# BaZzz01010101/ReflaxMan

Measured on AMD Instinct MI355X. Metric: Mrays/sec at 3840×2160 depth-8; max per-channel |Δ| vs CPU reference, higher is better.
Workload: dtype f32; 1 GPU; C3 synth16: 16 spheres + 4 textured triangles + sun, 3840x2160, depth 8, 1 spp; scene=synth16, width=3840, height=2160, depth=8, spp=1, parallelism=single-gpu

## Files before the change

### include/rfx.h

```cpp
#ifndef RFX_H
#define RFX_H
#include <stddef.h>
#include <stdint.h>

#ifdef __cplusplus
extern "C" {
#endif

#define RFX_ABI_VERSION 5

typedef enum {
  RFX_OK = 0,
  RFX_ERR_ARG = -1,
  RFX_ERR_HIP = -2,
  RFX_ERR_STATE = -3,
  RFX_ERR_IO = -4,
  RFX_ERR_RNG = -5,
  RFX_ERR_NODEV = -6
} rfx_status;

enum { RFX_METAL = 0, RFX_DIELECTRIC = 1 };

typedef struct rfx_scene rfx_scene;
typedef struct rfx_renderer rfx_renderer;
// ... 17 lines not shown
int rfx_scene_plane_count(const rfx_scene *scene);
int rfx_triangle_set_texture(rfx_scene *scene, int object_index, int texture_index, const float uv[6]);
int rfx_scene_add_light(rfx_scene *scene, const float origin[3], float radius, const float rgb[3], float power);
int rfx_scene_add_texture_argb(rfx_scene *scene, uint32_t width, uint32_t height, const uint32_t *argb);
int rfx_scene_add_texture_file(rfx_scene *scene, const char *path, int *loaded);
int rfx_scene_set_skybox_file(rfx_scene *scene, const char *path);
int rfx_scene_set_skybox_argb(rfx_scene *scene, uint32_t width, uint32_t height, const uint32_t *argb);
int rfx_scene_counts(const rfx_scene *scene, int *spheres, int *triangles, int *lights, int *textures);
int rfx_scene_tri_bvh_dump(const rfx_scene *scene, int32_t counts[5], float *boxes, int32_t *children,
                           int32_t *leaf_ids, int32_t *residual);
int rfx_scene_cull_dump(const rfx_scene *scene, float recs[64 * 8], float tris[32 * 12], uint64_t *valid);
int rfx_scene_set_tri_mates(rfx_scene *scene, int on);
int rfx_scene_tri_mates(const rfx_scene *scene, int32_t *leader, float *plane);
int rfx_scene_set_far_lights(rfx_scene *scene, int mode);
int rfx_scene_far_light(const rfx_scene *scene, int light, float terms[8]);

void rfx_camera_view(const float eye[3], const float at[3], float view[9]);
float rfx_camera_rz(uint32_t width, float fov);

int rfx_tga_load(const char *path, uint32_t *width, uint32_t *height, uint32_t *argb, size_t capacity);
int rfx_tga_save(const char *path, uint32_t width, uint32_t height, const uint32_t *argb);
int rfx_bmp_save(const char *path, uint32_t width, uint32_t height, const uint32_t *argb);
void rfx_argb_from_rgb(const float *rgb, size_t pixels, uint32_t *argb);

int rfx_renderer_create(rfx_renderer **out, int device);
void rfx_renderer_destroy(rfx_renderer *r);
int rfx_renderer_device(const rfx_renderer *r);
int rfx_renderer_set_stream(rfx_renderer *r, void *hip_stream);
int rfx_renderer_set_scene(rfx_renderer *r, const rfx_scene *scene);
int rfx_renderer_set_tile_order(rfx_renderer *r, int mode);
// ... 190 lines not shown
```

### reflaxman_amd/_lib.py

```python
from __future__ import annotations

import ctypes as C
import os

from . import _build

RFX_OK = 0
RFX_NCOUNTERS = 40
RFX_ABI_VERSION = 5
RFX_ORDER_CELL_BITS, RFX_ORDER_DIR_BITS, RFX_ORDER_TILE = 4, 10, 4096
RFX_TRI_RECORD_WORDS = 41
METAL, DIELECTRIC = 0, 1

_fp = C.POINTER(C.c_float)
_u32p = C.POINTER(C.c_uint32)
_u64p = C.POINTER(C.c_uint64)


class RfxError(RuntimeError):
    pass


class Frame(C.Structure):
    _fields_ = [
# ... 39 lines not shown

SIGNATURES = [
    ("rfx_abi_version", C.c_int, []),
    ("rfx_last_error", C.c_char_p, []),
    ("rfx_build_options", C.c_int, []),
    ("rfx_scene_create", C.c_void_p, [C.c_float] * 4),
    ("rfx_scene_destroy", None, [C.c_void_p]),
    ("rfx_scene_add_sphere", C.c_int, [C.c_void_p, _fp, C.c_float, C.c_int, _fp, C.c_float, C.c_float]),
    ("rfx_scene_add_triangle", C.c_int, [C.c_void_p, _fp, _fp, _fp, C.c_int, _fp, C.c_float, C.c_float]),
    ("rfx_scene_add_mesh", C.c_int, [C.c_void_p, _fp, C.c_uint32, _u32p, C.c_uint32, C.c_int, _fp, C.c_float, C.c_float]),
    ("rfx_scene_tri_bvh_dump", C.c_int, [C.c_void_p, _i32p, _fp, _i32p, _i32p, _i32p]),
    ("rfx_scene_cull_dump", C.c_int, [C.c_void_p, _fp, _fp, _u64p]),
    ("rfx_scene_set_tri_mates", C.c_int, [C.c_void_p, C.c_int]),
    ("rfx_scene_tri_mates", C.c_int, [C.c_void_p, _i32p, _fp]),
    ("rfx_scene_set_far_lights", C.c_int, [C.c_void_p, C.c_int]),
    ("rfx_scene_far_light", C.c_int, [C.c_void_p, C.c_int, _fp]),
    ("rfx_scene_add_plane", C.c_int, [C.c_void_p, _fp, _fp, C.c_int, _fp, C.c_float, C.c_float]),
    ("rfx_scene_plane_count", C.c_int, [C.c_void_p]),
    ("rfx_triangle_set_texture", C.c_int, [C.c_void_p, C.c_int, C.c_int, _fp]),
    ("rfx_scene_add_light", C.c_int, [C.c_void_p, _fp, C.c_float, _fp, C.c_float]),
    ("rfx_scene_add_texture_argb", C.c_int, [C.c_void_p, C.c_uint32, C.c_uint32, _u32p]),
    ("rfx_scene_add_texture_file", C.c_int, [C.c_void_p, C.c_char_p, C.POINTER(C.c_int)]),
    ("rfx_scene_set_skybox_file", C.c_int, [C.c_void_p, C.c_char_p]),
    ("rfx_scene_set_skybox_argb", C.c_int, [C.c_void_p, C.c_uint32, C.c_uint32, _u32p]),
    ("rfx_scene_counts", C.c_int, [C.c_void_p] + [C.POINTER(C.c_int)] * 4),
    ("rfx_camera_view", None, [_fp, _fp, _fp]),
    ("rfx_camera_rz", C.c_float, [C.c_uint32, C.c_float]),
    ("rfx_tga_load", C.c_int, [C.c_char_p, _u32p, _u32p, _u32p, C.c_size_t]),
    ("rfx_tga_save", C.c_int, [C.c_char_p, C.c_uint32, C.c_uint32, _u32p]),
    ("rfx_bmp_save", C.c_int, [C.c_char_p, C.c_uint32, C.c_uint32, _u32p]),
# ... 197 lines not shown
```

### reflaxman_amd/csrc/rfx_bounce.h

```cpp
#pragma once
#include <hip/hip_runtime.h>

#include <cstddef>
#include <type_traits>

#include "rfx_math.h"
#include "rfx_types.h"
#include "rfx_shade_inputs.h"
#include "rfx_queries.h"

#pragma clang fp contract(off)

namespace rfx {

struct Park {
  int after;
  QRay *queue;
  uint32_t *count;
  uint32_t trace, out;
  static constexpr bool kRefill = false;
  __device__ __forceinline__ void ids(uint32_t &t, uint32_t &o) const { t = trace; o = out; }
  __device__ __forceinline__ uint32_t *keys() const { return nullptr; }
  __device__ __forceinline__ BvhGlobal bvh() const { return BvhGlobal{}; }
};
// ... 48 lines not shown
}

__device__ __forceinline__ bool near_light(const LightRec &L, v3 d)
{
  return fabsf(d.x) < L.near && fabsf(d.y) < L.near && fabsf(d.z) < L.near;
}

__device__ __forceinline__ LightRec reread_light(const LightRec *l, uint64_t when)
{
  typedef const __attribute__((address_space(4))) LightRec *ConstLightPtr;
  ConstLightPtr p = (ConstLightPtr)l;
  asm("" : "+s"(p) : "s"(when));
  return *(const LightRec *)p;
}

template <bool STATS, bool CULL, bool MANYL, bool SMALL, bool PLANES, bool PARK, class PK, bool ONEL = false,
          bool TBVH = false, bool FARL = false>
__device__ __forceinline__ col trace_from(const DevScene &RFX_SCENE_PARAM, v3 origin, v3 ray, col mulc, col pix, int refl,
                                          int depth, v3 rd, const float *lut, Cnt &cnt, bool valid, const PK &park,
                                          bool &parked, const uint64_t *pm_tile = nullptr, bool pm_shadow = true)
{
#ifdef RFX_LAUNDER_SCENE
  const DevScene &S = S_in;
#endif
  static_assert(!FARL || (ONEL && SMALL && CULL && !MANYL && !STATS), "FARL: the small-scene one-light culling kernels");
  constexpr bool FAR_SHADE = FARL && (RFX_FAR_LIGHT == 1 || RFX_FAR_LIGHT == 2);
  constexpr bool FAR_CONE = FARL && (RFX_FAR_LIGHT == 1 || RFX_FAR_LIGHT == 3);
  bool seg0 = pm_tile != nullptr;
  parked = false;
  if (valid && refl == 0) RFX_CNT(C_RAYS);
  const Tabs<SMALL> T{S};
  bool alive = valid && refl < depth;
  int occ_hint = -1;
#ifdef RFX_DEBUG_SEGS
  int nseg = 0;
#endif
  RFX_PROF_BEGIN(P_SEG);
  while (__ballot(alive))
  {
#ifdef RFX_DEBUG_SEGS
    if (alive) ++nseg;
#endif
// ... 56 lines not shown
    MatRec m{0.0f, 0.0f, 0.0f, 0.0f};
    int diel = 0;
    v3 reflv = mk(0.0f, 0.0f, 0.0f);
    float rayLen = 0.0f, normLen = 0.0f, reflectLen = 0.0f;
    col sumL = mkc(0.0f, 0.0f, 0.0f), sumS = mkc(0.0f, 0.0f, 0.0f);
    for (int base = 0;; base += 32)
    {
      RFX_PROF_BEGIN(P_SHADOW);
      uint32_t lit = 0;
      const int nl = ONEL ? 1 : min(32, S.n_light - base);
      for (int q = 0; q < nl; ++q)
      {
        const LightRec L = S.lights[base + q];
        bool facing = false;
        v3 sray = mk(0.0f, 0.0f, 0.0f);
        if (hit)
        {
          RFX_CNT(C_L_EVAL);
          const v3 dtl = sub(mk(L.ox, L.oy, L.oz), drop);
          if (dot(dtl, norm) > kVerySmall)
          {
            RFX_CNT(C_L_FACING);
            facing = true;
            sray = add(dtl, mul(rd, L.radius));
          }
        }
        if (__ballot(facing))
        {
          if constexpr (SMALL)
          {
            uint64_t om = S.cull_valid;
            if constexpr (CULL)
            {
              if (!MANYL && seg0 && pm_shadow && q < kPrimLights)
                om = pm_tile[1 + q];
              else
              {
                Bundle SB;
                bool far_cone = false;
                if constexpr (FAR_CONE) far_cone = __ballot(facing && !near_light(L, drop)) == 0;
                if (far_cone) SB = make_bundle_far(drop, L, facing);
                else SB = make_bundle(drop, sray, facing);
                if (SB.ok) om = cull_small(T.cull(), S.cull_valid, SB);
                RFX_CULL_STAT(1, SB.ok, __ballot(facing), om, S.cull_valid);
              }
            }
            if (facing && !occluded_small<STATS, PLANES>(S, drop, sray, skip_sph, skip_tri, skip_pln, om, cnt))
              lit |= 1u << q;
          }
          else
// ... 173 lines not shown
          alive = false;
        }
      }
    }
    if constexpr (PK::kRefill) park.refill(alive, origin, ray, mulc, pix, refl, rd);
  }
  RFX_PROF_END(P_SEG);
#ifdef RFX_DEBUG_SEGS
  return mkc((float)nseg, 0.0f, 0.0f);
#else
  return pix;
#endif
}

template <bool STATS, bool CULL, bool MANYL, bool SMALL, bool PLANES, bool ONEL = false, bool TBVH = false,
          bool FARL = false>
__device__ __forceinline__ col trace(const DevScene &S, v3 origin, v3 ray, int depth, v3 rd, const float *lut,
                                     Cnt &cnt, bool valid, const uint64_t *pm_tile = nullptr, bool pm_shadow = true)
{
  bool parked;
  return trace_from<STATS, CULL, MANYL, SMALL, PLANES, false, Park, ONEL, TBVH, FARL>(S, origin, ray, mkc(1.0f, 1.0f, 1.0f), mkc(0.0f, 0.0f, 0.0f), 0,
                                                       depth, rd, lut, cnt, valid, Park{0, nullptr, nullptr, 0, 0},
                                                       parked, pm_tile, pm_shadow);
}

}
```

### reflaxman_amd/csrc/rfx_bundle.h

```cpp
#pragma once
#include <hip/hip_runtime.h>

#include "rfx_math.h"
#include "rfx_types.h"

#pragma clang fp contract(off)

namespace rfx {

constexpr float kCullRel = 2e-3f;

struct Bundle {
  float cx, cy, cz, rw;
  float ax, ay, az, cosa, sina;
  bool ok;
};

__device__ __forceinline__ float lane_bcast(float v, int lane)
{
  return __int_as_float(__builtin_amdgcn_readlane(__float_as_int(v), lane));
}

__device__ __forceinline__ float wave_max_nonneg(float v)
{
  uint32_t u = __float_as_uint(v);
  u = max(u, (uint32_t)__builtin_amdgcn_update_dpp(0, (int)u, 0x111, 0xf, 0xf, false));
  u = max(u, (uint32_t)__builtin_amdgcn_update_dpp(0, (int)u, 0x112, 0xf, 0xf, false));
  u = max(u, (uint32_t)__builtin_amdgcn_update_dpp(0, (int)u, 0x114, 0xf, 0xf, false));
  u = max(u, (uint32_t)__builtin_amdgcn_update_dpp(0, (int)u, 0x118, 0xf, 0xf, false));
  u = max(u, (uint32_t)__builtin_amdgcn_update_dpp(0, (int)u, 0x142, 0xa, 0xf, false));
  u = max(u, (uint32_t)__builtin_amdgcn_update_dpp(0, (int)u, 0x143, 0xc, 0xf, false));
  return __int_as_float(__builtin_amdgcn_readlane((int)u, 63));
}

__device__ __forceinline__ float cdot(float ax, float ay, float az, float bx, float by, float bz)
{
#if RFX_CULL_FMA
  return __builtin_fmaf(az, bz, __builtin_fmaf(ay, by, ax * bx));
#else
  return ax * bx + ay * by + az * bz;
#endif
}

__device__ __forceinline__ Bundle make_bundle(v3 o, v3 d, bool live)
{
  Bundle B;
  const int ref = __ffsll((long long)__ballot(live)) - 1;
  B.cx = lane_bcast(o.x, ref); B.cy = lane_bcast(o.y, ref); B.cz = lane_bcast(o.z, ref);
  const float dx = lane_bcast(d.x, ref), dy = lane_bcast(d.y, ref), dz = lane_bcast(d.z, ref);
  const float inv = __builtin_amdgcn_rsqf(cdot(dx, dy, dz, dx, dy, dz));
  B.ax = dx * inv; B.ay = dy * inv; B.az = dz * inv;
  const float ex = o.x - B.cx, ey = o.y - B.cy, ez = o.z - B.cz;
  const float e2 = cdot(ex, ey, ez, ex, ey, ez);
  const float cosl = cdot(d.x, d.y, d.z, B.ax, B.ay, B.az) * __builtin_amdgcn_rsqf(cdot(d.x, d.y, d.z, d.x, d.y, d.z));
  const float dev = 1.0f - cosl;
  const bool bad = live && !(e2 <= 1.0e30f && dev >= -0.5f && dev <= 2.5f);
// ... 116 lines not shown
  const float px = B.cx + tp * B.ax - q.v0x, py = B.cy + tp * B.ay - q.v0y, pz = B.cz + tp * B.az - q.v0z;
  const float chord = __builtin_amdgcn_sqrtf(fmaxf(2.0f - 2.0f * B.cosa, 0.0f)) * 1.001f;
  const float R = (h * chord * (1.0f + ian) * ind + B.rw * (1.0f + ind) + 1e-4f * tp) * 1.001f + 1e-6f;
  const float cvx = B.cx - q.v0x, cvy = B.cy - q.v0y, cvz = B.cz - q.v0z;
  const float mag = __builtin_amdgcn_sqrtf(cvx * cvx + cvy * cvy + cvz * cvz) * 1.001f + B.rw + (h + B.rw) * ind;
  const float m = 1e-2f * mag + 1e-6f;
  const float u0 = q.gux * px + q.guy * py + q.guz * pz, v0 = q.gvx * px + q.gvy * py + q.gvz * pz;
  return u0 + (R + m) * q.nu < 0.0f || v0 + (R + m) * q.nv < 0.0f ||
         u0 + v0 - R * q.nuv - m * (q.nu + q.nv) > 1.0f;
}

template <bool FOOT = false>
__device__ __forceinline__ uint64_t cull_small(const CullRec *tab, uint64_t valid, const Bundle &B,
                                               const CullTri *ttab = nullptr)
{
  const CullRec g = tab[threadIdx.x & 63u];
  const float vx = g.x - B.cx, vy = g.y - B.cy, vz = g.z - B.cz;
  const float L2 = cdot(vx, vy, vz, vx, vy, vz);
  const float L = __builtin_amdgcn_sqrtf(L2);
#if RFX_CULL_FMA
  const float rp = __builtin_fmaf(kCullRel, L + B.rw, g.r + B.rw);
  const float va = cdot(vx, vy, vz, B.ax, B.ay, B.az);
  const float lim = __builtin_fmaf(B.cosa, __builtin_amdgcn_sqrtf(fmaxf(__builtin_fmaf(-rp, rp, L2), 0.0f)), -(B.sina * rp));
#else
  const float rp = g.r + B.rw + kCullRel * (L + B.rw);
  const float va = cdot(vx, vy, vz, B.ax, B.ay, B.az);
  const float lim = B.cosa * __builtin_amdgcn_sqrtf(fmaxf(L2 - rp * rp, 0.0f)) - B.sina * rp;
#endif
  const float side = cdot(g.nx, g.ny, g.nz, B.cx, B.cy, B.cz) - g.d;
  const float an = cdot(g.nx, g.ny, g.nz, B.ax, B.ay, B.az);
  const float ms = B.rw + 1e-3f * (L + g.r + B.rw) + 1e-6f, ma = B.sina + 1e-3f;
  const bool away = (side > ms && an > ma) || (side < -ms && an < -ma);
  bool keep = !(L > rp && va < lim) && !away;
  if constexpr (FOOT)
    if ((threadIdx.x & 63u) >= 32u && keep) keep = !tri_footprint_misses(ttab[(threadIdx.x & 63u) - 32u], side, an, B);
  return __ballot(keep) & valid;
}

__device__ __forceinline__ uint64_t all_bits(int n) { return n >= 64 ? ~0ull : ((1ull << n) - 1ull); }

__device__ __forceinline__ uint32_t pair_bits(uint64_t m)
{
  uint64_t x = (m | (m >> 1)) & 0x5555555555555555ull;
  x = (x | (x >> 1)) & 0x3333333333333333ull;
  x = (x | (x >> 2)) & 0x0F0F0F0F0F0F0F0Full;
  x = (x | (x >> 4)) & 0x00FF00FF00FF00FFull;
  x = (x | (x >> 8)) & 0x0000FFFF0000FFFFull;
  x = (x | (x >> 16)) & 0x00000000FFFFFFFFull;
  return (uint32_t)x;
}
// ... 3 lines not shown
```

### reflaxman_amd/csrc/rfx_config.h

```cpp
#pragma once

#ifndef RFX_DIV_FAST
#define RFX_DIV_FAST 1
#endif
#ifndef RFX_DIV_SINGLE
#define RFX_DIV_SINGLE 0
#endif

#ifndef RFX_BVH_LEAF_PAIRS
#define RFX_BVH_LEAF_PAIRS 4
#endif
#ifndef RFX_TRI_BVH
#define RFX_TRI_BVH 1
#endif
#ifndef RFX_TRI_BVH_LEAF
#define RFX_TRI_BVH_LEAF 4
#endif
#ifndef RFX_TRI_BVH_AUTO_MIN
#define RFX_TRI_BVH_AUTO_MIN 128
#endif
#ifndef RFX_TRI_BVH_NARROW_MIN
#define RFX_TRI_BVH_NARROW_MIN (1 << 30)
#endif

#if !defined(RFX_WAVES_PER_EU) && defined(RFX_LANES_WAVES_PER_EU) && defined(RFX_UNIT_LANES_FAST)
#define RFX_WAVES_PER_EU RFX_LANES_WAVES_PER_EU
#endif
#ifndef RFX_WAVES_PER_EU
#define RFX_WAVES_PER_EU 7
#endif
#ifndef RFX_WG_WAVES
#define RFX_WG_WAVES 2
#endif
#ifndef RFX_TRI_MATES
#define RFX_TRI_MATES 2
#endif
#ifndef RFX_FAR_LIGHT
#define RFX_FAR_LIGHT 1
#endif
#ifndef RFX_CULL_FMA
#define RFX_CULL_FMA 1
#endif
#ifndef RFX_NARROW_BUNDLE_COS
#define RFX_NARROW_BUNDLE_COS 0.9995f
#endif
#ifndef RFX_OCC_HINT
#define RFX_OCC_HINT 1
#endif
#ifndef RFX_ONE_LIGHT
#define RFX_ONE_LIGHT 1
#endif
#ifndef RFX_SSAA_LANES
#define RFX_SSAA_LANES 1
// ... 81 lines not shown
```

### reflaxman_amd/csrc/rfx_host.cpp

```cpp
#include <string.h>

#include <algorithm>

#include "rfx_internal.h"
#include "rfx_math.h"

#pragma clang fp contract(off)

using namespace rfx;

extern "C" int rfx_abi_version(void) { return RFX_ABI_VERSION; }

constexpr uint64_t kMaxLaunchTraces = 1ull << 31;

static int timing_event(rfx_renderer *r, hipStream_t st)
{
  if (!r->timing_this) return RFX_OK;
  if (r->events_used == r->events.size())
  {
    hipEvent_t e;
    HIP_CHECK(hipEventCreate(&e));
    r->events.push_back(e);
  }
  HIP_CHECK(hipEventRecord(r->events[r->events_used++], st));
// ... 238 lines not shown
{
  if (!r || !s) return fail(RFX_ERR_ARG, "set_scene: bad args");
  int rc;
  if ((rc = set_dev(r)) != RFX_OK) return rc;
  HIP_CHECK(hipStreamSynchronize(r->stream));
  free_scene(r);
  const SceneBuild B(*s, r->tri_accel);
  DevScene d = B.d;
  if ((rc = upload(r, B.sg, &d.sph_geo)) || (rc = upload(r, B.sp, &d.sph_pair)) || (rc = upload(r, B.sm, &d.sph_mat)) ||
      (rc = upload(r, B.si, &d.sph_info)) || (rc = upload(r, B.tg, &d.tri_geo)) || (rc = upload(r, B.ts, &d.tri_shade)) ||
      (rc = upload(r, B.tm, &d.tri_mat)) || (rc = upload(r, B.lr, &d.lights)) || (rc = upload(r, B.tr, &d.texs)) ||
      (rc = upload(r, B.pool, &d.texels)) || (rc = upload(r, B.bd, &d.bound)) || (rc = upload(r, B.cs, &d.cull_small)) ||
      (rc = upload(r, B.ct, &d.cull_tri)) || (rc = upload(r, B.cb, &d.chunk_bound)) || (rc = upload(r, B.pg, &d.pln_geo)) ||
      (rc = upload(r, B.pm, &d.pln_mat)) || (rc = upload(r, B.loc, &d.obj_loc)) || (rc = upload(r, B.bvh, &d.bvh)) ||
      (rc = upload(r, B.tt.nodes, &d.tri_bvh)) || (rc = upload(r, B.tleaf, &d.tri_leaf)) ||
      (rc = upload(r, B.tt.resid, &d.tri_resid)) || (rc = upload(r, B.aux, &d.bvh_aux)))
    return rc;
  r->dev = d;
  if ((rc = upload_update_tables(r, B)) != RFX_OK) return rc;
  r->accel = B.accel;
  r->order_box = B.order_box;
  r->dev = d;
  r->has_scene = true;
  ++r->scene_gen;
  r->prim_key.clear();
  r->prim_seen.clear();
  return RFX_OK;
}

extern "C" int rfx_renderer_set_rng(rfx_renderer *r, uint32_t sphere_seed, uint32_t jitter_seed)
{
// ... 820 lines not shown
```

### reflaxman_amd/csrc/rfx_scene.cpp

```cpp
#include <math.h>
#include <stdarg.h>
#include <stdio.h>
#include <stdlib.h>
#include <string.h>

#include <algorithm>
#include <array>
#include <cmath>
#include <map>
#include <string>
#include <vector>

#include "rfx_math.h"
#include "rfx_refit.h"
#include "rfx_scene.h"

#pragma clang fp contract(off)

using namespace rfx;

static thread_local std::string g_last_error;

int rfx::fail(int code, const char *fmt, ...)
{
  char buf[512];
  va_list ap;
  va_start(ap, fmt);
// ... 15 lines not shown
  float tu0 = 0, tv0 = 0;
  int tex = -1;
  HostMat mat;
  int obj;
};
struct HostLight { v3 origin; float radius; float r, g, b, power; };
struct HostPlane { v3 pos, norm; HostMat mat; int obj; };

struct rfx_scene {
  col diff, env;
  float diff_power;
  float half_tile_w, half_tile_h;
  int skybox = -1;
  int tri_mates = 1;
  int far_lights = 1;
  std::vector<HostSphere> spheres;
  std::vector<HostTri> tris;
  std::vector<HostPlane> planes;
  std::vector<int> obj_kind, obj_idx;
  std::vector<HostLight> lights;
  std::vector<HostTexture> textures;
};

static void default_half_tiles(rfx_scene *s)
{
  s->half_tile_w = 1.0f / 8.0f - kFltEpsilon;
  s->half_tile_h = 1.0f / 6.0f - kFltEpsilon;
}

extern "C" rfx_scene *rfx_scene_create(float dr, float dg, float db, float dp)
{
  rfx_scene *s = new rfx_scene();
  s->diff = mkc(dr, dg, db);
  s->diff_power = dp;
  s->env = cscale(s->diff, dp);
  default_half_tiles(s);
  return s;
}

extern "C" void rfx_scene_destroy(rfx_scene *s) { delete s; }

static HostMat make_mat(int type, const float rgb[3], float refl, float transp)
{
  HostMat m;
  m.dielectric = type == RFX_DIELECTRIC;
  m.r = rgb[0]; m.g = rgb[1]; m.b = rgb[2];
  m.refl = clampf(refl, 0.0f, 1.0f);
  m.transp = clampf(transp, 0.0f, 1.0f);
  return m;
}

// ... 596 lines not shown

extern "C" int rfx_scene_set_far_lights(rfx_scene *s, int mode)
{
  if (!s || mode < 0 || mode > 2) return fail(RFX_ERR_ARG, "scene_set_far_lights: 0 (off), 1 (auto) or 2 (any extent)");
  s->far_lights = mode;
  return RFX_OK;
}

extern "C" int rfx_scene_far_light(const rfx_scene *s, int light, float terms[8])
{
  if (!s || light < 0 || light >= (int)s->lights.size()) return fail(RFX_ERR_ARG, "scene_far_light: no light %d", light);
  const LightRec rec = far_light_terms(s->lights[light]);
  if (terms)
    for (float f : {rec.dlen, rec.ndx, rec.ndy, rec.ndz, rec.spec_add, rec.near, rec.cone_cos, rec.cone_sin}) *terms++ = f;
  return far_light_scene(*s, rec) ? 1 : 0;
}

static OrderBox order_box_of(const rfx_scene &s)
{
  float lo[3] = {INFINITY, INFINITY, INFINITY}, hi[3] = {-INFINITY, -INFINITY, -INFINITY};
  const auto take = [&](int a, float l, float h) {
    if (l < lo[a]) lo[a] = l;
    if (h > hi[a]) hi[a] = h;
  };
  for (size_t k = 0; k < s.obj_kind.size(); ++k)
  {
    if (s.obj_kind[k] == 0)
    {
      const HostSphere &h = s.spheres[s.obj_idx[k]];
      const float c[3] = {h.center.x, h.center.y, h.center.z};
// ... 293 lines not shown
    const float lo[3] = {fminf(root.lx[0], root.lx[1]), fminf(root.ly[0], root.ly[1]), fminf(root.lz[0], root.lz[1])};
    const float hi[3] = {fmaxf(root.hx[0], root.hx[1]), fmaxf(root.hy[0], root.hy[1]), fmaxf(root.hz[0], root.hz[1])};
    float s[3];
    for (int k = 0; k < 3; ++k) s[k] = hi[k] > lo[k] ? 8.0f / (hi[k] - lo[k]) : 0.0f;
    d.key_lx = lo[0]; d.key_ly = lo[1]; d.key_lz = lo[2];
    d.key_sx = s[0]; d.key_sy = s[1]; d.key_sz = s[2];
  }
  d.n_obj = (int32_t)loc.size();
  d.cull_valid = cull_valid;
  d.skybox_tex = s->skybox;
  const col amb = cscale(s->diff, s->diff_power);
  d.amb_r = amb.r; d.amb_g = amb.g; d.amb_b = amb.b;
  d.env_r = s->env.r; d.env_g = s->env.g; d.env_b = s->env.b;
  d.half_tile_w = s->half_tile_w;
  d.half_tile_h = s->half_tile_h;
}

extern "C" int rfx_scene_cull_dump(const rfx_scene *s, float recs[64 * 8], float tris[32 * 12], uint64_t *valid)
{
  if (!s) return fail(RFX_ERR_ARG, "scene_cull_dump: no scene");
  if (!(s->spheres.size() <= 32 && s->tris.size() <= 32))
    return fail(RFX_ERR_STATE, "scene_cull_dump: not a small scene (more than 32 spheres or triangles)");
  const SceneBuild B(*s, 0);
  static_assert(sizeof(CullRec) == 8 * sizeof(float) && sizeof(CullTri) == 12 * sizeof(float), "dump layout");
  if (recs) memcpy(recs, B.cs.data(), 64 * sizeof(CullRec));
  if (tris) memcpy(tris, B.ct.data(), 32 * sizeof(CullTri));
  if (valid) *valid = B.d.cull_valid;
  return RFX_OK;
}

// ... 108 lines not shown
```

### reflaxman_amd/csrc/rfx_scene.h

```cpp
#pragma once
#include <stdint.h>

#include <vector>

#include "../../include/rfx.h"
#include "rfx_types.h"
#include "rfx_order_types.h"

namespace rfx {

int fail(int code, const char *fmt, ...) __attribute__((format(printf, 2, 3)));

struct TriTree {
  std::vector<BvhNode> nodes;
  std::vector<int32_t> order;
  std::vector<int32_t> resid;
  int depth = 0;
  size_t leaves() const { return order.size() / RFX_TRI_BVH_LEAF; }
};

struct SceneBuild {
  SceneBuild(const rfx_scene &scene, int tri_accel);
  std::vector<SphereGeo> sg;
  std::vector<SpherePair> sp;
  std::vector<MatRec> sm, tm, pm;
  std::vector<int32_t> si, loc;
  std::vector<TriGeo> tg, tleaf;
  std::vector<TriShade> ts;
  std::vector<Bound> bd, cb;
  std::vector<CullRec> cs;
  std::vector<CullTri> ct;
  std::vector<BvhNode> bvh;
  std::vector<uint32_t> aux, pool;
  TriTree tt;
  std::vector<PlaneGeo> pg;
  std::vector<LightRec> lr;
  std::vector<TexRec> tr;
  DevScene d{};
  rfx_accel_info accel{};
  OrderBox order_box{};
  std::vector<float> tverts;
  std::vector<int32_t> tslot, hlist;
  std::vector<uint32_t> till, hoff;
};

void tri_record_words(uint32_t *out, const TriGeo &g, const TriShade &h, const Bound &b, const float *verts9, bool well,
// ... 4 lines not shown
```

### reflaxman_amd/csrc/rfx_trace.h

```cpp
#pragma once
#include <hip/hip_runtime.h>

#include "rfx_math.h"
#include "rfx_launch.h"
#include "rfx_types.h"
#include "rfx_shade_inputs.h"
#include "rfx_bounce.h"

#pragma clang fp contract(off)

namespace rfx {

template <bool STATS>
__device__ __forceinline__ void flush_counters(const FrameParams &P, Cnt &cnt)
{
  if constexpr (STATS)
  {
#pragma unroll
    for (int k = 0; k < C_COUNT; ++k)
    {
      unsigned long long v = cnt.c[k];
#pragma unroll
      for (int off = 32; off > 0; off >>= 1) v += __shfl_xor(v, off, 64);
      if ((threadIdx.x & 63) == 0 && v) atomicAdd(&P.counters[k], v);
// ... 171 lines not shown
      float rndx = 0.0f, rndy = 0.0f;
      if (P.additive && valid)
      {
        const uint32_t s1 = lcg_jump(P.jitter_seed, 2 * pr + 1);
        rndx = (float)lcg_out(s1) / (float)0x7FFF;
        rndy = (float)lcg_out(lcg_step(s1)) / (float)0x7FFF;
      }
      const float ssf = (float)(int)ss;
      const float ox = sx ? (float)(int)sx / ssf : 0.0f, oy = sy ? (float)(int)sy / ssf : 0.0f;
      const float rx = (float)x - P.wh, ry = (float)y - P.hh;
      const v3 ray = mmul(view, mk(rx + ox + rndx, ry + oy + rndy, P.rz));
      v3 rd = mk(0.0f, 0.0f, 0.0f);
      if (valid) rd = load_rd(P, pr * (uint64_t)ss2 + kk);
      const uint64_t *pm = RFX_PRIM_LANES && SMALL && CULL && !STATS && P.prim_mask
                               ? P.prim_mask + (size_t)kPrimStride * t8 : nullptr;
      const col c = trace<STATS, CULL, MANYL, SMALL, PLANES, ONEL, TBVH, FARL>(S, eye, ray, P.depth, rd, lut, cnt, valid, pm,
                                                                        P.prim_shadow != 0);
      {
#ifdef RFX_LAUNDER_PARAMS
        const FrameParams &P = kernarg_params();
#endif
        const uint32_t t8e = ((volatile uint32_t *)s_tile8)[wv];
        uint32_t le = lane;
        asm volatile("" : "+v"(le));
        const uint32_t ss = (uint32_t)P.ss, ss2 = ss * ss, bw = CHUNKS ? 1u : ss_lane_block(P.ss);
        const uint32_t q = bw == 1 ? 0 : le / ss2, kk = bw == 1 ? 64 * chunk + le : le - q * ss2;
        const uint32_t lx = (t8e % w8) * bw + q % bw, ly = (t8e / w8) * bw + q / bw;
        const uint32_t x = lx;
        const uint32_t y = P.nranks > 1 ? strip_row_to_y(ly, P) : ly + P.row0;
        const uint64_t p = (uint64_t)y * P.W + x;
        const bool pvalid = lx < P.W && ly < P.grid_rows && p >= P.p_begin && p < P.p_end;
// ... 94 lines not shown
    const uint32_t x = gx;
    const uint32_t y = P.nranks > 1 ? strip_row_to_y(gy, P) : gy + P.row0;
    const uint64_t p = (uint64_t)y * P.W + x;
    const bool valid = gx < P.W && gy < P.grid_rows && p >= P.p_begin && p < P.p_end;
    const uint64_t pr = p - P.p_begin;
    const float rx = (float)x - P.wh, ry = (float)y - P.hh;
    col out;
    bool parked = false;
    if constexpr (MODE == kModePlain)
    {
      const v3 ray = mmul(view, mk(rx + 0.0f + 0.0f, ry + 0.0f + 0.0f, P.rz));
      v3 rd = mk(0.0f, 0.0f, 0.0f);
      if (valid) rd = load_rd(P, pr);
      const ParkTile park{P.park_after, P.queue, P.queue_count, P, wv, w8};
      const uint64_t *pm_tile = SMALL && CULL && !STATS && P.prim_mask ? P.prim_mask + (size_t)kPrimStride * t8 : nullptr;
      const col c = trace_from<STATS, CULL, MANYL, SMALL, PLANES, PARK, ParkTile, ONEL, TBVH, FARL>(
          S, eye, ray, mkc(1.0f, 1.0f, 1.0f), mkc(0.0f, 0.0f, 0.0f), 0, P.depth, rd, lut, cnt, valid, park, parked, pm_tile);
      out = cadd(mkc(0.0f, 0.0f, 0.0f), c);
    }
    else
    {
      float rndx = 0.0f, rndy = 0.0f;
      if (P.additive && valid)
      {
        const uint32_t s1 = lcg_jump(P.jitter_seed, 2 * pr + 1);
        rndx = (float)lcg_out(s1) / (float)0x7FFF;
        rndy = (float)lcg_out(lcg_step(s1)) / (float)0x7FFF;
      }
      const int ss = P.ss;
      const float ssf = (float)ss;
      col fin = mkc(0.0f, 0.0f, 0.0f);
// ... 124 lines not shown
```

### reflaxman_amd/csrc/rfx_types.h

```cpp
#pragma once
#include "rfx_config.h"

#include <stddef.h>
#include <stdint.h>

namespace rfx {

enum Counter {
  C_RAYS = 0, C_SEGMENTS,
  C_SPH_TESTS, C_SPH_B, C_SPH_D, C_SPH_T,
  C_TRI_TESTS, C_TRI_Z, C_TRI_S, C_TRI_T, C_TRI_IN, C_TRI_D,
  C_HIT_SPH, C_HIT_TRI,
  C_SH_SPH_TESTS, C_SH_SPH_B, C_SH_SPH_D, C_SH_SPH_T,
  C_SH_TRI_TESTS, C_SH_TRI_Z, C_SH_TRI_S, C_SH_TRI_T, C_SH_TRI_IN,
  C_L_EVAL, C_L_FACING, C_L_LIT, C_L_SPEC, C_L_POW,
  C_DIELECTRIC, C_METAL, C_CONTINUE, C_SKY,
  C_TEX_BILINEAR, C_TEX_CHECKER, C_TEX_OTHER,
  C_PLN_TESTS, C_PLN_T, C_HIT_PLN, C_SH_PLN_TESTS, C_SH_PLN_T,
  C_COUNT
};

struct alignas(16) SphereGeo { float cx, cy, cz, sq_radius; };
struct alignas(32) SpherePair { float cx[2], cy[2], cz[2], r2[2]; };
struct alignas(16) MatRec { float r, g, b, refl; };
// ... 6 lines not shown
  float nx, ny, nz, tu0;
  float t11, t12, t21, t22;
  float tv0; int32_t tex; int32_t dielectric; int32_t obj;
};
struct alignas(16) Bound { float x, y, z, r; };
struct alignas(16) CullRec { float x, y, z, r, nx, ny, nz, d; };
struct alignas(16) CullTri { float v0x, v0y, v0z, nu, gux, guy, guz, nv, gvx, gvy, gvz, nuv; };
constexpr int kBvhStack = 16;
struct alignas(16) BvhNode { float lx[2], ly[2], lz[2], hx[2], hy[2], hz[2]; int32_t child[2]; float mt[2]; };
struct alignas(16) PlaneGeo { float px, py, pz, nx, ny, nz; int32_t obj, dielectric; };
struct alignas(16) LightRec {
  float ox, oy, oz, radius, r, g, b, power;
  float dlen, ndx, ndy, ndz, spec_add, near, cone_cos, cone_sin;
};
struct alignas(16) TexRec { uint32_t offset, w, h, pad; };

struct DevScene {
  const SphereGeo *sph_geo;
  const SpherePair *sph_pair;
  const MatRec *sph_mat;
  const int32_t *sph_info;
  const TriGeo *tri_geo;
  const TriShade *tri_shade;
  const MatRec *tri_mat;
  const LightRec *lights;
  const TexRec *texs;
  const uint32_t *texels;
  const Bound *bound;
  const Bound *chunk_bound;
  const BvhNode *bvh;
// ... 12 lines not shown
  int32_t n_chunk;
  const uint32_t *bvh_aux;
  float bvh_mstep;
  int32_t n_bvh;
  float amb_r, amb_g, amb_b;
  float env_r, env_g, env_b;
  float half_tile_w, half_tile_h;
  const BvhNode *tri_bvh;
  const TriGeo *tri_leaf;
  const int32_t *tri_resid;
  int32_t n_tri_resid;
  int32_t n_tri_bvh;
  int32_t tri_bvh_depth;
  int32_t tri_bvh_narrow;
  int32_t far_light;
};

constexpr int kLdsBvhWaves = 16, kLdsBvhStackSlots = 16;
constexpr size_t lds_bvh_bytes(int n_bvh)
{
  return (size_t)n_bvh * 56 + sizeof(int16_t) * kLdsBvhStackSlots * 64 * kLdsBvhWaves + 4 * 64 * kLdsBvhWaves;
}
constexpr bool lds_bvh_fits(int n_bvh) { return n_bvh > 0 && lds_bvh_bytes(n_bvh) + 4096 <= 160 * 1024; }

constexpr uint32_t kQueueBuckets = 4096;
struct alignas(16) QRay {
  float ox, oy, oz, dx;
  float dy, dz, mr, mg;
  float mb, pr, pg, pb;
  uint32_t trace, out, refl, pad;
// ... 49 lines not shown
```

### reflaxman_amd/render.py

```python
from __future__ import annotations

import contextlib
import ctypes as C
import os
from typing import List, Optional, Sequence

import numpy as np

from . import _lib
from ._lib import DIELECTRIC, METAL, check, farr

DEFAULT_SPHERE_SEED = 1350490027
DEFAULT_JITTER_SEED = 424238335


class Vector3:
    __slots__ = ("x", "y", "z")

    def __init__(self, x=0.0, y=0.0, z=0.0):
        self.x, self.y, self.z = float(x), float(y), float(z)

    def __iter__(self):
        return iter((self.x, self.y, self.z))

# ... 171 lines not shown
    def tri_mates(self, plane: bool = False):
        L = _lib.load()
        n = check(L.rfx_scene_tri_mates(self._h, None, None), "Scene.tri_mates")
        leader, rows = np.zeros(n, np.int32), np.zeros((n, 6), np.float32)
        check(L.rfx_scene_tri_mates(self._h, leader.ctypes.data_as(_lib._i32p), _lib.fptr(rows)), "Scene.tri_mates")
        return (leader, rows) if plane else leader

    def set_far_lights(self, mode: int):
        check(_lib.load().rfx_scene_set_far_lights(self._h, int(mode)), "Scene.set_far_lights")
        self._version += 1

    def far_light(self, light: int = 0):
        terms = np.zeros(8, np.float32)
        chosen = check(_lib.load().rfx_scene_far_light(self._h, int(light), _lib.fptr(terms)), "Scene.far_light")
        return bool(chosen), terms

    def addPlane(self, pos: Vector3, norm: Vector3, material: Material) -> Plane:
        obj = check(_lib.load().rfx_scene_add_plane(self._h, farr(Vector3(*pos)), farr(Vector3(*norm)), material.type,
                                                    farr(material.color), material.reflectivity, material.transparency),
                    "Scene.addPlane")
        self._version += 1
        return Plane(self, obj)

    def addLight(self, origin: Vector3, radius: float, color: Color, power: float) -> OmniLight:
        idx = check(_lib.load().rfx_scene_add_light(self._h, farr(Vector3(*origin)), float(radius), farr(Color(*color)),
                                                    float(power)), "Scene.addLight")
        self._version += 1
        return OmniLight(self, idx)

    def addTexture(self, fileName: str) -> Texture:
# ... 920 lines not shown
```

Before: 14390 Mrays/s.

## Precompute per-cell shadow cull masks in a spatial grid for the far light

Builds a host-side 3D grid over the scene bounds. Each cell stores a 64-bit mask of cull records that a shadow cone from anywhere in that cell toward the single far light could hit, computed with a conservative ball radius. In the non-parked tile kernel, when every facing lane in a wave falls in the grid and is outside the light's near region, the shadow mask is an OR of the cell masks instead of a bundle build plus per-record cull test. This adds a global memory gather per hit and a coarser, more conservative mask, which can mean more shadow candidates per wave and extra scene-build time on the host.

```diff
diff --git a/include/rfx.h b/include/rfx.h
--- a/include/rfx.h
+++ b/include/rfx.h
@@ -55,6 +55,8 @@
 int rfx_scene_tri_mates(const rfx_scene *scene, int32_t *leader, float *plane);
 int rfx_scene_set_far_lights(rfx_scene *scene, int mode);
 int rfx_scene_far_light(const rfx_scene *scene, int light, float terms[8]);
+int rfx_scene_set_shadow_grid(rfx_scene *scene, int mode);
+int rfx_scene_shadow_grid(const rfx_scene *scene, float geom[6], int32_t dims[3], uint64_t *masks, uint64_t capacity);
 
 void rfx_camera_view(const float eye[3], const float at[3], float view[9]);
 float rfx_camera_rz(uint32_t width, float fov);
diff --git a/reflaxman_amd/_lib.py b/reflaxman_amd/_lib.py
--- a/reflaxman_amd/_lib.py
+++ b/reflaxman_amd/_lib.py
@@ -77,6 +77,8 @@
     ("rfx_scene_set_tri_mates", C.c_int, [C.c_void_p, C.c_int]),
     ("rfx_scene_tri_mates", C.c_int, [C.c_void_p, _i32p, _fp]),
     ("rfx_scene_set_far_lights", C.c_int, [C.c_void_p, C.c_int]),
+    ("rfx_scene_set_shadow_grid", C.c_int, [C.c_void_p, C.c_int]),
+    ("rfx_scene_shadow_grid", C.c_int, [C.c_void_p, _fp, _i32p, _u64p, C.c_uint64]),
     ("rfx_scene_far_light", C.c_int, [C.c_void_p, C.c_int, _fp]),
     ("rfx_scene_add_plane", C.c_int, [C.c_void_p, _fp, _fp, C.c_int, _fp, C.c_float, C.c_float]),
     ("rfx_scene_plane_count", C.c_int, [C.c_void_p]),
diff --git a/reflaxman_amd/csrc/rfx_bounce.h b/reflaxman_amd/csrc/rfx_bounce.h
--- a/reflaxman_amd/csrc/rfx_bounce.h
+++ b/reflaxman_amd/csrc/rfx_bounce.h
@@ -4,6 +4,7 @@
 #include <cstddef>
 #include <type_traits>
 
+#include "rfx_cull_rule.h"
 #include "rfx_math.h"
 #include "rfx_types.h"
 #include "rfx_shade_inputs.h"
@@ -86,8 +87,16 @@
   return *(const LightRec *)p;
 }
 
+__device__ __forceinline__ ShadowGrid reread_grid(uint64_t when)
+{
+  typedef const __attribute__((address_space(4))) char *KP;
+  KP p = (KP)__builtin_amdgcn_kernarg_segment_ptr();
+  asm("" : "+s"(p) : "s"(when));
+  return *(const ShadowGrid *)(const __attribute__((address_space(4))) ShadowGrid *)(p + offsetof(DevScene, shadow_grid));
+}
+
 template <bool STATS, bool CULL, bool MANYL, bool SMALL, bool PLANES, bool PARK, class PK, bool ONEL = false,
-          bool TBVH = false, bool FARL = false>
+          bool TBVH = false, bool FARL = false, bool SGRID = FARL>
 __device__ __forceinline__ col trace_from(const DevScene &RFX_SCENE_PARAM, v3 origin, v3 ray, col mulc, col pix, int refl,
                                           int depth, v3 rd, const float *lut, Cnt &cnt, bool valid, const PK &park,
                                           bool &parked, const uint64_t *pm_tile = nullptr, bool pm_shadow = true)
@@ -98,6 +107,8 @@
   static_assert(!FARL || (ONEL && SMALL && CULL && !MANYL && !STATS), "FARL: the small-scene one-light culling kernels");
   constexpr bool FAR_SHADE = FARL && (RFX_FAR_LIGHT == 1 || RFX_FAR_LIGHT == 2);
   constexpr bool FAR_CONE = FARL && (RFX_FAR_LIGHT == 1 || RFX_FAR_LIGHT == 3);
+  constexpr bool GRID = FAR_CONE && SGRID && RFX_SHADOW_GRID != 0;
+  constexpr bool GRID_EARLY = GRID && RFX_SHADOW_GRID != 2;
   bool seg0 = pm_tile != nullptr;
   parked = false;
   if (valid && refl == 0) RFX_CNT(C_RAYS);
@@ -184,6 +195,17 @@
         const LightRec L = S.lights[base + q];
         bool facing = false;
         v3 sray = mk(0.0f, 0.0f, 0.0f);
+        ShadowGrid G{};
+        bool in_grid = false;
+        int32_t cell = 0;
+        uint64_t cell_mask = 0;
+        if constexpr (GRID)
+        {
+          G = reread_grid(__ballot(hit));
+          in_grid = shadow_grid_cell(G, drop.x, drop.y, drop.z, &cell) & hit & (G.cells != nullptr) & !(seg0 && pm_shadow);
+          if constexpr (GRID_EARLY)
+            if (in_grid) cell_mask = G.cells[cell];
+        }
         if (hit)
         {
           RFX_CNT(C_L_EVAL);
@@ -204,6 +226,13 @@
             {
               if (!MANYL && seg0 && pm_shadow && q < kPrimLights)
                 om = pm_tile[1 + q];
+              else if (GRID && __ballot(facing & !(in_grid & near_light(L, drop))) == 0)
+              {
+                if constexpr (!GRID_EARLY)
+                  if (facing) cell_mask = G.cells[cell];
+                om = wave_or(facing ? cell_mask : 0ull) & S.cull_valid;
+                RFX_CULL_STAT(1, true, __ballot(facing), om, S.cull_valid);
+              }
               else
               {
                 Bundle SB;
@@ -407,12 +436,12 @@
 }
 
 template <bool STATS, bool CULL, bool MANYL, bool SMALL, bool PLANES, bool ONEL = false, bool TBVH = false,
-          bool FARL = false>
+          bool FARL = false, bool SGRID = FARL>
 __device__ __forceinline__ col trace(const DevScene &S, v3 origin, v3 ray, int depth, v3 rd, const float *lut,
                                      Cnt &cnt, bool valid, const uint64_t *pm_tile = nullptr, bool pm_shadow = true)
 {
   bool parked;
-  return trace_from<STATS, CULL, MANYL, SMALL, PLANES, false, Park, ONEL, TBVH, FARL>(S, origin, ray, mkc(1.0f, 1.0f, 1.0f), mkc(0.0f, 0.0f, 0.0f), 0,
+  return trace_from<STATS, CULL, MANYL, SMALL, PLANES, false, Park, ONEL, TBVH, FARL, SGRID>(S, origin, ray, mkc(1.0f, 1.0f, 1.0f), mkc(0.0f, 0.0f, 0.0f), 0,
                                                        depth, rd, lut, cnt, valid, Park{0, nullptr, nullptr, 0, 0},
                                                        parked, pm_tile, pm_shadow);
 }
diff --git a/reflaxman_amd/csrc/rfx_bundle.h b/reflaxman_amd/csrc/rfx_bundle.h
--- a/reflaxman_amd/csrc/rfx_bundle.h
+++ b/reflaxman_amd/csrc/rfx_bundle.h
@@ -1,20 +1,13 @@
 #pragma once
 #include <hip/hip_runtime.h>
 
+#include "rfx_cull_rule.h"
 #include "rfx_math.h"
 #include "rfx_types.h"
 
 #pragma clang fp contract(off)
 
 namespace rfx {
-
-constexpr float kCullRel = 2e-3f;
-
-struct Bundle {
-  float cx, cy, cz, rw;
-  float ax, ay, az, cosa, sina;
-  bool ok;
-};
 
 __device__ __forceinline__ float lane_bcast(float v, int lane)
 {
@@ -33,13 +26,19 @@
   return __int_as_float(__builtin_amdgcn_readlane((int)u, 63));
 }
 
-__device__ __forceinline__ float cdot(float ax, float ay, float az, float bx, float by, float bz)
-{
-#if RFX_CULL_FMA
-  return __builtin_fmaf(az, bz, __builtin_fmaf(ay, by, ax * bx));
-#else
-  return ax * bx + ay * by + az * bz;
-#endif
+__device__ __forceinline__ uint32_t wave_or32(uint32_t u)
+{
+  u |= (uint32_t)__builtin_amdgcn_update_dpp(0, (int)u, 0x111, 0xf, 0xf, false);
+  u |= (uint32_t)__builtin_amdgcn_update_dpp(0, (int)u, 0x112, 0xf, 0xf, false);
+  u |= (uint32_t)__builtin_amdgcn_update_dpp(0, (int)u, 0x114, 0xf, 0xf, false);
+  u |= (uint32_t)__builtin_amdgcn_update_dpp(0, (int)u, 0x118, 0xf, 0xf, false);
+  u |= (uint32_t)__builtin_amdgcn_update_dpp(0, (int)u, 0x142, 0xa, 0xf, false);
+  u |= (uint32_t)__builtin_amdgcn_update_dpp(0, (int)u, 0x143, 0xc, 0xf, false);
+  return (uint32_t)__builtin_amdgcn_readlane((int)u, 63);
+}
+__device__ __forceinline__ uint64_t wave_or(uint64_t m)
+{
+  return (uint64_t)wave_or32((uint32_t)(m >> 32)) << 32 | wave_or32((uint32_t)m);
 }
 
 __device__ __forceinline__ Bundle make_bundle(v3 o, v3 d, bool live)
@@ -186,26 +185,10 @@
 __device__ __forceinline__ uint64_t cull_small(const CullRec *tab, uint64_t valid, const Bundle &B,
                                                const CullTri *ttab = nullptr)
 {
-  const CullRec g = tab[threadIdx.x & 63u];
-  const float vx = g.x - B.cx, vy = g.y - B.cy, vz = g.z - B.cz;
-  const float L2 = cdot(vx, vy, vz, vx, vy, vz);
-  const float L = __builtin_amdgcn_sqrtf(L2);
-#if RFX_CULL_FMA
-  const float rp = __builtin_fmaf(kCullRel, L + B.rw, g.r + B.rw);
-  const float va = cdot(vx, vy, vz, B.ax, B.ay, B.az);
-  const float lim = __builtin_fmaf(B.cosa, __builtin_amdgcn_sqrtf(fmaxf(__builtin_fmaf(-rp, rp, L2), 0.0f)), -(B.sina * rp));
-#else
-  const float rp = g.r + B.rw + kCullRel * (L + B.rw);
-  const float va = cdot(vx, vy, vz, B.ax, B.ay, B.az);
-  const float lim = B.cosa * __builtin_amdgcn_sqrtf(fmaxf(L2 - rp * rp, 0.0f)) - B.sina * rp;
-#endif
-  const float side = cdot(g.nx, g.ny, g.nz, B.cx, B.cy, B.cz) - g.d;
-  const float an = cdot(g.nx, g.ny, g.nz, B.ax, B.ay, B.az);
-  const float ms = B.rw + 1e-3f * (L + g.r + B.rw) + 1e-6f, ma = B.sina + 1e-3f;
-  const bool away = (side > ms && an > ma) || (side < -ms && an < -ma);
-  bool keep = !(L > rp && va < lim) && !away;
+  const CullVerdict v = cull_record(tab[threadIdx.x & 63u], B);
+  bool keep = v.keep;
   if constexpr (FOOT)
-    if ((threadIdx.x & 63u) >= 32u && keep) keep = !tri_footprint_misses(ttab[(threadIdx.x & 63u) - 32u], side, an, B);
+    if ((threadIdx.x & 63u) >= 32u && keep) keep = !tri_footprint_misses(ttab[(threadIdx.x & 63u) - 32u], v.side, v.an, B);
   return __ballot(keep) & valid;
 }
 
diff --git a/reflaxman_amd/csrc/rfx_config.h b/reflaxman_amd/csrc/rfx_config.h
--- a/reflaxman_amd/csrc/rfx_config.h
+++ b/reflaxman_amd/csrc/rfx_config.h
@@ -37,6 +37,12 @@
 #endif
 #ifndef RFX_FAR_LIGHT
 #define RFX_FAR_LIGHT 1
+#endif
+#ifndef RFX_SHADOW_GRID
+#define RFX_SHADOW_GRID 1
+#endif
+#ifndef RFX_SHADOW_GRID_CELLS
+#define RFX_SHADOW_GRID_CELLS (1 << 16)
 #endif
 #ifndef RFX_CULL_FMA
 #define RFX_CULL_FMA 1
diff --git a/reflaxman_amd/csrc/rfx_cull_rule.h b/reflaxman_amd/csrc/rfx_cull_rule.h
--- /dev/null
+++ b/reflaxman_amd/csrc/rfx_cull_rule.h
@@ -0,0 +1,67 @@
+#pragma once
+#include "rfx_math.h"
+#include "rfx_types.h"
+
+#pragma clang fp contract(off)
+
+namespace rfx {
+
+constexpr float kCullRel = 2e-3f;
+
+struct Bundle {
+  float cx, cy, cz, rw;
+  float ax, ay, az, cosa, sina;
+  bool ok;
+};
+
+RFX_HD float cull_sqrt(float x)
+{
+#if defined(__HIP_DEVICE_COMPILE__)
+  return __builtin_amdgcn_sqrtf(x);
+#else
+  return sqrtf(x);
+#endif
+}
+
+RFX_HD float cdot(float ax, float ay, float az, float bx, float by, float bz)
+{
+#if RFX_CULL_FMA
+  return __builtin_fmaf(az, bz, __builtin_fmaf(ay, by, ax * bx));
+#else
+  return ax * bx + ay * by + az * bz;
+#endif
+}
+
+struct CullVerdict { bool keep; float side, an; };
+RFX_HD CullVerdict cull_record(const CullRec &g, const Bundle &B)
+{
+  const float vx = g.x - B.cx, vy = g.y - B.cy, vz = g.z - B.cz;
+  const float L2 = cdot(vx, vy, vz, vx, vy, vz);
+  const float L = cull_sqrt(L2);
+#if RFX_CULL_FMA
+  const float rp = __builtin_fmaf(kCullRel, L + B.rw, g.r + B.rw);
+  const float va = cdot(vx, vy, vz, B.ax, B.ay, B.az);
+  const float lim = __builtin_fmaf(B.cosa, cull_sqrt(fmaxf(__builtin_fmaf(-rp, rp, L2), 0.0f)), -(B.sina * rp));
+#else
+  const float rp = g.r + B.rw + kCullRel * (L + B.rw);
+  const float va = cdot(vx, vy, vz, B.ax, B.ay, B.az);
+  const float lim = B.cosa * cull_sqrt(fmaxf(L2 - rp * rp, 0.0f)) - B.sina * rp;
+#endif
+  CullVerdict v;
+  v.side = cdot(g.nx, g.ny, g.nz, B.cx, B.cy, B.cz) - g.d;
+  v.an = cdot(g.nx, g.ny, g.nz, B.ax, B.ay, B.az);
+  const float ms = B.rw + 1e-3f * (L + g.r + B.rw) + 1e-6f, ma = B.sina + 1e-3f;
+  const bool away = (v.side > ms && v.an > ma) || (v.side < -ms && v.an < -ma);
+  v.keep = !(L > rp && va < lim) && !away;
+  return v;
+}
+
+RFX_HD bool shadow_grid_cell(const ShadowGrid &G, float px, float py, float pz, int32_t *cell)
+{
+  const float fx = (px - G.ox) * G.scale, fy = (py - G.oy) * G.scale, fz = (pz - G.oz) * G.scale;
+  const bool in = (fx >= 0.0f) & (fx < G.fnx) & (fy >= 0.0f) & (fy < G.fny) & (fz >= 0.0f) & (fz < G.fnz);
+  *cell = in ? ((int32_t)fz * G.ny + (int32_t)fy) * G.nx + (int32_t)fx : 0;
+  return in;
+}
+
+}
diff --git a/reflaxman_amd/csrc/rfx_host.cpp b/reflaxman_amd/csrc/rfx_host.cpp
--- a/reflaxman_amd/csrc/rfx_host.cpp
+++ b/reflaxman_amd/csrc/rfx_host.cpp
@@ -276,7 +276,8 @@
       (rc = upload(r, B.ct, &d.cull_tri)) || (rc = upload(r, B.cb, &d.chunk_bound)) || (rc = upload(r, B.pg, &d.pln_geo)) ||
       (rc = upload(r, B.pm, &d.pln_mat)) || (rc = upload(r, B.loc, &d.obj_loc)) || (rc = upload(r, B.bvh, &d.bvh)) ||
       (rc = upload(r, B.tt.nodes, &d.tri_bvh)) || (rc = upload(r, B.tleaf, &d.tri_leaf)) ||
-      (rc = upload(r, B.tt.resid, &d.tri_resid)) || (rc = upload(r, B.aux, &d.bvh_aux)))
+      (rc = upload(r, B.tt.resid, &d.tri_resid)) || (rc = upload(r, B.aux, &d.bvh_aux)) ||
+      (rc = upload(r, B.gm, &d.shadow_grid.cells)))
     return rc;
   r->dev = d;
   if ((rc = upload_update_tables(r, B)) != RFX_OK) return rc;
diff --git a/reflaxman_amd/csrc/rfx_scene.cpp b/reflaxman_amd/csrc/rfx_scene.cpp
--- a/reflaxman_amd/csrc/rfx_scene.cpp
+++ b/reflaxman_amd/csrc/rfx_scene.cpp
@@ -11,6 +11,7 @@
 #include <string>
 #include <vector>
 
+#include "rfx_cull_rule.h"
 #include "rfx_math.h"
 #include "rfx_refit.h"
 #include "rfx_scene.h"
@@ -56,6 +57,7 @@
   int skybox = -1;
   int tri_mates = 1;
   int far_lights = 1;
+  int shadow_grid = 1;
   std::vector<HostSphere> spheres;
   std::vector<HostTri> tris;
   std::vector<HostPlane> planes;
@@ -77,6 +79,8 @@
   s->diff_power = dp;
   s->env = cscale(s->diff, dp);
   default_half_tiles(s);
+  if (const char *v = getenv("RFX_SHADOW_GRID"))
+    if ((v[0] == '0' || v[0] == '1' || v[0] == '2') && !v[1]) s->shadow_grid = v[0] - '0';
   return s;
 }
 
@@ -703,6 +707,125 @@
   if (terms)
     for (float f : {rec.dlen, rec.ndx, rec.ndy, rec.ndz, rec.spec_add, rec.near, rec.cone_cos, rec.cone_sin}) *terms++ = f;
   return far_light_scene(*s, rec) ? 1 : 0;
+}
+
+constexpr double kGridBoxMargin = 1.0 / 1024.0;
+
+static bool shadow_grid_scene(const rfx_scene &s, const LightRec &rec, bool small)
+{
+  if (!RFX_SHADOW_GRID || s.shadow_grid == 0 || !small || s.lights.size() != 1 || !(rec.near > 0.0f)) return false;
+  return s.shadow_grid == 2 || far_light_scene(s, rec);
+}
+
+static void shadow_grid_build(const rfx_scene &s, const LightRec &light, SceneBuild &B)
+{
+  double lo[3] = {INFINITY, INFINITY, INFINITY}, hi[3] = {-INFINITY, -INFINITY, -INFINITY};
+  const auto take = [&](int a, double l, double h) { lo[a] = fmin(lo[a], l); hi[a] = fmax(hi[a], h); };
+  for (const HostSphere &h : s.spheres)
+  {
+    const double c[3] = {h.center.x, h.center.y, h.center.z};
+    for (int a = 0; a < 3; ++a) take(a, c[a] - h.radius, c[a] + h.radius);
+  }
+  for (const HostTri &t : s.tris)
+    for (const v3 *v : {&t.v0, &t.v1, &t.v2}) { take(0, v->x, v->x); take(1, v->y, v->y); take(2, v->z, v->z); }
+  double edge = 0.0;
+  for (int a = 0; a < 3; ++a)
+  {
+    if (!std::isfinite(lo[a]) || !std::isfinite(hi[a])) return;
+    edge = fmax(edge, hi[a] - lo[a]);
+  }
+  if (!(edge > 0.0) || !(edge < 1.0e30)) return;
+  float flo[3];
+  double ext[3], cmax = 0.0;
+  for (int a = 0; a < 3; ++a)
+  {
+    flo[a] = (float)(lo[a] - kGridBoxMargin * edge);
+    if ((double)flo[a] > lo[a] - kGridBoxMargin * edge) flo[a] = nextafterf(flo[a], -INFINITY);
+    ext[a] = hi[a] + kGridBoxMargin * edge - (double)flo[a];
+  }
+  const auto cells = [&](double size, int32_t n[3]) {
+    double total = 1.0;
+    for (int a = 0; a < 3; ++a)
+    {
+      const double c = fmax(1.0, ceil(ext[a] / size));
+      n[a] = c < 1.0e9 ? (int32_t)c : 1000000000;
+      total *= c;
+    }
+    return total;
+  };
+  const double budget = (double)RFX_SHADOW_GRID_CELLS;
+  int32_t n[3];
+  double fits = fmax(ext[0], fmax(ext[1], ext[2])), over = cbrt(ext[0] * ext[1] * ext[2] / budget) * 0.5;
+  if (cells(over, n) <= budget) fits = over;
+  else
+    for (int it = 0; it < 60; ++it)
+    {
+      const double mid = 0.5 * (fits + over);
+      (cells(mid, n) <= budget ? fits : over) = mid;
+    }
+  float size = (float)fits;
+  if ((double)size < fits) size = nextafterf(size, INFINITY);
+  while (cells((double)size, n) > budget) size = nextafterf(size * 1.000001f, INFINITY);
+  const float scale = 1.0f / size;
+  if (!(size > 0.0f) || !std::isfinite(size) || !std::isfinite(scale) || !(scale > 0.0f)) return;
+  for (int a = 0; a < 3; ++a) cmax = fmax(cmax, fmax(fabs((double)flo[a]), fabs((double)flo[a] + (double)n[a] * size)));
+  const int32_t nmax = std::max(n[0], std::max(n[1], n[2]));
+  const double ball = 0.5 * sqrt(3.0) * (double)size * (1.0 + 1.0e-6 * nmax + 1.0e-5) + 2.5e-7 * cmax;
+  float rw = (float)ball;
+  if ((double)rw < ball) rw = nextafterf(rw, INFINITY);
+  Bundle cone{};
+  cone.rw = rw;
+  cone.ax = light.ndx; cone.ay = light.ndy; cone.az = light.ndz;
+  cone.cosa = light.cone_cos; cone.sina = light.cone_sin;
+  cone.ok = true;
+  std::vector<int> lanes;
+  for (int l = 0; l < 64; ++l)
+    if ((B.d.cull_valid >> l) & 1u) lanes.push_back(l);
+  B.gm.assign((size_t)n[0] * n[1] * n[2], 0ull);
+  size_t k = 0;
+  for (int32_t iz = 0; iz < n[2]; ++iz)
+    for (int32_t iy = 0; iy < n[1]; ++iy)
+      for (int32_t ix = 0; ix < n[0]; ++ix, ++k)
+      {
+        cone.cx = (float)((double)flo[0] + (ix + 0.5) * (double)size);
+        cone.cy = (float)((double)flo[1] + (iy + 0.5) * (double)size);
+        cone.cz = (float)((double)flo[2] + (iz + 0.5) * (double)size);
+        uint64_t m = 0;
+        for (int l : lanes)
+          if (cull_record(B.cs[l], cone).keep) m |= 1ull << l;
+        B.gm[k] = m;
+      }
+  ShadowGrid &g = B.d.shadow_grid;
+  g.ox = flo[0]; g.oy = flo[1]; g.oz = flo[2];
+  g.scale = scale;
+  g.nx = n[0]; g.ny = n[1]; g.nz = n[2];
+  g.fnx = (float)n[0]; g.fny = (float)n[1]; g.fnz = (float)n[2];
+  B.grid_cell = size;
+  B.grid_ball = rw;
+}
+
+extern "C" int rfx_scene_set_shadow_grid(rfx_scene *s, int mode)
+{
+  if (!s || mode < 0 || mode > 2) return fail(RFX_ERR_ARG, "scene_set_shadow_grid: 0 (off), 1 (auto) or 2 (any far light)");
+  s->shadow_grid = mode;
+  return RFX_OK;
+}
+
+extern "C" int rfx_scene_shadow_grid(const rfx_scene *s, float geom[6], int32_t dims[3], uint64_t *masks, uint64_t capacity)
+{
+  if (!s) return fail(RFX_ERR_ARG, "scene_shadow_grid: no scene");
+  const SceneBuild B(*s, 0);
+  const ShadowGrid &g = B.d.shadow_grid;
+  if (geom)
+    for (float f : {g.ox, g.oy, g.oz, g.scale, B.grid_cell, B.grid_ball}) *geom++ = f;
+  if (dims)
+    for (int32_t v : {g.nx, g.ny, g.nz}) *dims++ = v;
+  if (masks)
+  {
+    if (capacity < B.gm.size()) return fail(RFX_ERR_ARG, "scene_shadow_grid: room for %zu masks needed", B.gm.size());
+    if (!B.gm.empty()) memcpy(masks, B.gm.data(), B.gm.size() * sizeof(uint64_t));
+  }
+  return (int)B.gm.size();
 }
 
 static OrderBox order_box_of(const rfx_scene &s)
@@ -1026,6 +1149,7 @@
   d.env_r = s->env.r; d.env_g = s->env.g; d.env_b = s->env.b;
   d.half_tile_w = s->half_tile_w;
   d.half_tile_h = s->half_tile_h;
+  if (!lr.empty() && shadow_grid_scene(*s, lr[0], small)) shadow_grid_build(*s, lr[0], *this);
 }
 
 extern "C" int rfx_scene_cull_dump(const rfx_scene *s, float recs[64 * 8], float tris[32 * 12], uint64_t *valid)
diff --git a/reflaxman_amd/csrc/rfx_scene.h b/reflaxman_amd/csrc/rfx_scene.h
--- a/reflaxman_amd/csrc/rfx_scene.h
+++ b/reflaxman_amd/csrc/rfx_scene.h
@@ -30,6 +30,8 @@
   std::vector<Bound> bd, cb;
   std::vector<CullRec> cs;
   std::vector<CullTri> ct;
+  std::vector<uint64_t> gm;
+  float grid_cell = 0, grid_ball = 0;
   std::vector<BvhNode> bvh;
   std::vector<uint32_t> aux, pool;
   TriTree tt;
diff --git a/reflaxman_amd/csrc/rfx_trace.h b/reflaxman_amd/csrc/rfx_trace.h
--- a/reflaxman_amd/csrc/rfx_trace.h
+++ b/reflaxman_amd/csrc/rfx_trace.h
@@ -209,7 +209,7 @@
       if (valid) rd = load_rd(P, pr * (uint64_t)ss2 + kk);
       const uint64_t *pm = RFX_PRIM_LANES && SMALL && CULL && !STATS && P.prim_mask
                                ? P.prim_mask + (size_t)kPrimStride * t8 : nullptr;
-      const col c = trace<STATS, CULL, MANYL, SMALL, PLANES, ONEL, TBVH, FARL>(S, eye, ray, P.depth, rd, lut, cnt, valid, pm,
+      const col c = trace<STATS, CULL, MANYL, SMALL, PLANES, ONEL, TBVH, FARL, false>(S, eye, ray, P.depth, rd, lut, cnt, valid, pm,
                                                                         P.prim_shadow != 0);
       {
 #ifdef RFX_LAUNDER_PARAMS
@@ -334,7 +334,7 @@
       if (valid) rd = load_rd(P, pr);
       const ParkTile park{P.park_after, P.queue, P.queue_count, P, wv, w8};
       const uint64_t *pm_tile = SMALL && CULL && !STATS && P.prim_mask ? P.prim_mask + (size_t)kPrimStride * t8 : nullptr;
-      const col c = trace_from<STATS, CULL, MANYL, SMALL, PLANES, PARK, ParkTile, ONEL, TBVH, FARL>(
+      const col c = trace_from<STATS, CULL, MANYL, SMALL, PLANES, PARK, ParkTile, ONEL, TBVH, FARL, FARL && !PARK>(
           S, eye, ray, mkc(1.0f, 1.0f, 1.0f), mkc(0.0f, 0.0f, 0.0f), 0, P.depth, rd, lut, cnt, valid, park, parked, pm_tile);
       out = cadd(mkc(0.0f, 0.0f, 0.0f), c);
     }
diff --git a/reflaxman_amd/csrc/rfx_types.h b/reflaxman_amd/csrc/rfx_types.h
--- a/reflaxman_amd/csrc/rfx_types.h
+++ b/reflaxman_amd/csrc/rfx_types.h
@@ -44,6 +44,12 @@
   float dlen, ndx, ndy, ndz, spec_add, near, cone_cos, cone_sin;
 };
 struct alignas(16) TexRec { uint32_t offset, w, h, pad; };
+struct ShadowGrid {
+  const uint64_t *cells;
+  float ox, oy, oz, scale;
+  float fnx, fny, fnz;
+  int32_t nx, ny, nz;
+};
 
 struct DevScene {
   const SphereGeo *sph_geo;
@@ -86,6 +92,7 @@
   int32_t tri_bvh_depth;
   int32_t tri_bvh_narrow;
   int32_t far_light;
+  ShadowGrid shadow_grid;
 };
 
 constexpr int kLdsBvhWaves = 16, kLdsBvhStackSlots = 16;
diff --git a/reflaxman_amd/render.py b/reflaxman_amd/render.py
--- a/reflaxman_amd/render.py
+++ b/reflaxman_amd/render.py
@@ -209,6 +209,22 @@
         terms = np.zeros(8, np.float32)
         chosen = check(_lib.load().rfx_scene_far_light(self._h, int(light), _lib.fptr(terms)), "Scene.far_light")
         return bool(chosen), terms
+
+    def set_shadow_grid(self, mode: int):
+        check(_lib.load().rfx_scene_set_shadow_grid(self._h, int(mode)), "Scene.set_shadow_grid")
+        self._version += 1
+
+    def shadow_grid(self):
+        L = _lib.load()
+        n = check(L.rfx_scene_shadow_grid(self._h, None, None, None, 0), "Scene.shadow_grid")
+        if n == 0:
+            return None
+        geom, dims, masks = np.zeros(6, np.float32), np.zeros(3, np.int32), np.zeros(n, np.uint64)
+        check(L.rfx_scene_shadow_grid(self._h, _lib.fptr(geom), dims.ctypes.data_as(_lib._i32p), _lib.u64ptr(masks), n),
+              "Scene.shadow_grid")
+        nx, ny, nz = (int(v) for v in dims)
+        return {"origin": geom[:3].copy(), "scale": geom[3], "cell": geom[4], "ball": geom[5], "dims": (nx, ny, nz),
+                "masks": masks.reshape(nz, ny, nx)}
 
     def addPlane(self, pos: Vector3, norm: Vector3, material: Material) -> Plane:
         obj = check(_lib.load().rfx_scene_add_plane(self._h, farr(Vector3(*pos)), farr(Vector3(*norm)), material.type,
```

Result: faster. 14910 Mrays/s (median of 6 runs) (+3.6%).
